# ishine/TargetDiarization

Measured on AMD Instinct MI355X. Metric: real-time factor (audio-sec/wall-sec) full infer() pipe, 16kHz mono, 1/2/4/8 GPU, higher is better.
Workload: dtype f32 (split-f16 x3: fp32-accurate products from three f16 MFMA passes, fp32 accumulate); 1 GPU; BASELINE configs[3]: 1800 s synthetic conversation (two alternating speakers, 20 % overlap) = 180 x 10 s windows: MossFormer2 (90 windows per launch) -> loudness swap -> ERes2NetV2 on every 10 s window of both streams + cosine vs a target embedding -> Paraformer (SANM encoder, CIF predictor, NAR decoder, argmax tokens + timestamps) on 30 s segments of both streams -> CT-Transformer punctuation of ; windows_per_launch=90

## Files before the change

### targetdiarization_amd/csrc/gemm_h3.hpp

```cpp
#pragma once
#include <cstdio>
#include <cstdlib>
#include <typeinfo>
#include <vector>
#include <hip/hip_runtime.h>
#include <stdint.h>

#include "devutil.hpp"
#include "gemm.hpp"

namespace tdx {

typedef _Float16 f16x8 __attribute__((ext_vector_type(8)));

constexpr int H3_BM = 256, H3_BN = 256, H3_BK = 16, H3_THREADS = 512;
constexpr int H3_ROWB = 64;
constexpr int H3_OPER = 256 * H3_ROWB;
constexpr int H3_STAGE = 2 * H3_OPER;
constexpr int H3_NBUF = 4;
constexpr int H3_AUX_AHEAD = 3;
constexpr int H3_LDS = H3_NBUF * H3_STAGE;
constexpr int H3_LDS_EXTRA = 12288;

struct H3Seg {
    const unsigned char* A;
    const unsigned char* B;
    const float* sa;
    const float* sb;
    long lda, ldb;
    long strideA, strideB, strideA2, strideB2;
    long strideSA, strideSB, strideSA2, strideSB2;
    int sa_mul, sb_mul;
    int K;
    int zdiv;
    int kchunk, ktotal;
    int segk;
    long strideSeg;
    int a_shift, a_period;
    const unsigned char* a_zero;
};

struct H3Args {
    H3Seg seg[2];
    int nseg;
    int M, N;
    int tiles_m, tiles_n;
    int map_mode, mp, gw, batches;
    int mc;
    int pair_off;
    int cv_Hin, cv_Win, cv_Hout, cv_Wout, cv_stride, cv_ntaps, cv_cin;
    int cv_taps_total;
    const unsigned char* zero_row;
    int dbg;
    unsigned long long* stamps;
};

#ifdef TDX_H3_STAMPS
#define H3_STAMP(i) do { if (g.stamps && threadIdx.x == 0) g.stamps[(long)blockIdx.x * 8 + (i)] = wall_clock64(); } while (0)
#define H3_STAMP_HW() do { if (g.stamps && threadIdx.x == 0) g.stamps[(long)blockIdx.x * 8 + 7] = \
    (unsigned long long)__builtin_amdgcn_s_getreg((31 << 11) | 4) | ((unsigned long long)__builtin_amdgcn_s_getreg((31 << 11) | 20) << 32); } while (0)
#else
#define H3_STAMP(i) do {} while (0)
#define H3_STAMP_HW() do {} while (0)
#endif

inline H3Seg h3_seg(const void* A, const float* sa, long lda, const void* B, const float* sb, long ldb, int K) {
    H3Seg s{};
    s.A = (const unsigned char*)A; s.B = (const unsigned char*)B; s.sa = sa; s.sb = sb; s.lda = lda; s.ldb = ldb; s.K = K; s.zdiv = 1;
    s.sa_mul = 1; s.sb_mul = 1;
    return s;
}

__device__ __forceinline__ void h3_glds16(const unsigned char* g, unsigned char* l) {
    __builtin_amdgcn_global_load_lds((const __attribute__((address_space(1))) void*)g, (__attribute__((address_space(3))) void*)l, 16, 0, 0);
}

typedef __fp16 h3_fp16x4 __attribute__((__vector_size__(4 * sizeof(__fp16))));
typedef _Float16 f16x4 __attribute__((ext_vector_type(4)));

template <bool TR>
__device__ __forceinline__ f16x8 h3_frag(const unsigned char* p) {
    if constexpr (!TR) {
        return *reinterpret_cast<const f16x8*>(p);
    } else {
        const h3_fp16x4 lo = __builtin_amdgcn_ds_read_tr16_b64_v4f16((__attribute__((address_space(3))) h3_fp16x4*)p);
        const h3_fp16x4 hi = __builtin_amdgcn_ds_read_tr16_b64_v4f16((__attribute__((address_space(3))) h3_fp16x4*)(p + 4096));
        f16x8 r;
#pragma unroll
        for (int i = 0; i < 4; ++i) { r[i] = (_Float16)lo[i]; r[4 + i] = (_Float16)hi[i]; }
        return r;
    }
}

struct H3TrRaw { uint2 lo, hi; };
__device__ __forceinline__ unsigned h3_lds_addr(const unsigned char* p) {
    return (unsigned)(size_t)(__attribute__((address_space(3))) const unsigned char*)p;
}
template <int OFF>
__device__ __forceinline__ void h3_tr_read(H3TrRaw& r, unsigned a) {
    asm volatile("ds_read_b64_tr_b16 %0, %1 offset:%2" : "=v"(r.lo) : "v"(a), "n"(OFF) : "memory");
    asm volatile("ds_read_b64_tr_b16 %0, %1 offset:%2" : "=v"(r.hi) : "v"(a), "n"(OFF + 4096) : "memory");
}
__device__ __forceinline__ f16x8 h3_tr_value(const H3TrRaw& r) {
    typedef unsigned u4 __attribute__((ext_vector_type(4)));
    return __builtin_bit_cast(f16x8, u4{r.lo.x, r.lo.y, r.hi.x, r.hi.y});
}
template <int N>
__device__ __forceinline__ void h3_tr_fence(H3TrRaw (&r)[N]) {
    static_assert(N == 2 || N == 4 || N == 8, "fence over 2, 4 or 8 raw fragments");
    if constexpr (N == 8)
        asm volatile("s_waitcnt lgkmcnt(0)" : "+v"(r[0].lo), "+v"(r[0].hi), "+v"(r[1].lo), "+v"(r[1].hi), "+v"(r[2].lo), "+v"(r[2].hi), "+v"(r[3].lo), "+v"(r[3].hi),
                     "+v"(r[4].lo), "+v"(r[4].hi), "+v"(r[5].lo), "+v"(r[5].hi), "+v"(r[6].lo), "+v"(r[6].hi), "+v"(r[7].lo), "+v"(r[7].hi) :: "memory");
    else if constexpr (N == 4)
        asm volatile("s_waitcnt lgkmcnt(0)" : "+v"(r[0].lo), "+v"(r[0].hi), "+v"(r[1].lo), "+v"(r[1].hi), "+v"(r[2].lo), "+v"(r[2].hi), "+v"(r[3].lo), "+v"(r[3].hi) :: "memory");
    else
        asm volatile("s_waitcnt lgkmcnt(0)" : "+v"(r[0].lo), "+v"(r[0].hi), "+v"(r[1].lo), "+v"(r[1].hi) :: "memory");
}
// ... 116 lines not shown
        const _Float16 a = (_Float16)xs;
        hi[i] = a;
        lo[i] = (_Float16)(xs - (float)a);
    }
    *reinterpret_cast<f16x8*>(dst) = hi;
    *reinterpret_cast<f16x8*>(dst + 16) = lo;
}

struct H3Pair { uint2 hi, lo; };
__device__ __forceinline__ H3Pair h3_split4(float4 v, float s) {
    typedef _Float16 h4 __attribute__((ext_vector_type(4)));
    const float xs[4] = {v.x * s, v.y * s, v.z * s, v.w * s};
    h4 a, b;
#pragma unroll
    for (int j = 0; j < 4; ++j) { const _Float16 t = (_Float16)xs[j]; a[j] = t; b[j] = (_Float16)(xs[j] - (float)t); }
    H3Pair r;
    r.hi = __builtin_bit_cast(uint2, a); r.lo = __builtin_bit_cast(uint2, b);
    return r;
}
__device__ __forceinline__ uint4 h3_pair16(int q, float4 v, float s) {
    const H3Pair o = h3_split4(v, s);
    const bool odd = q & 1;
    const uint2 send = odd ? o.hi : o.lo;
    uint2 recv;
    recv.x = (unsigned)__builtin_amdgcn_mov_dpp((int)send.x, 0xB1, 0xF, 0xF, true);
    recv.y = (unsigned)__builtin_amdgcn_mov_dpp((int)send.y, 0xB1, 0xF, 0xF, true);
    return odd ? make_uint4(recv.x, recv.y, o.lo.x, o.lo.y) : make_uint4(o.hi.x, o.hi.y, recv.x, recv.y);
}
__device__ __forceinline__ void h3_emit4(unsigned char* prow, int q, float4 v, float s) {
    *reinterpret_cast<uint4*>(prow + (q >> 1) * 32 + ((q & 1) ? 16 : 0)) = h3_pair16(q, v, s);
}
__device__ __forceinline__ void h3_emit4_pred(unsigned char* prow, int q, float4 v, float s, bool ok) {
    const uint4 w = h3_pair16(q, v, s);
    if (ok) *reinterpret_cast<uint4*>(prow + (q >> 1) * 32 + ((q & 1) ? 16 : 0)) = w;
}
__device__ __forceinline__ float h3_absmax4(float4 v) { return fmaxf(fmaxf(fabsf(v.x), fabsf(v.y)), fmaxf(fabsf(v.z), fabsf(v.w))); }


struct H3PlOut { unsigned char* planes; long pitch; float* scale; float* ss; long seg_stride; };
template <class E, class = void> struct epi_has_plout { static constexpr bool value = false; };
template <class E> struct epi_has_plout<E, decltype((void)&E::plout, void())> { static constexpr bool value = true; };
template <class E, class = void> struct epi_has_rowout { static constexpr bool value = false; };
template <class E> struct epi_has_rowout<E, decltype((void)&E::rowout, void())> { static constexpr bool value = true; };
struct H3Conv {
    const float* w; int wld;
    int ncols;
    unsigned char* planes; long pitch;
    float sv;
    float* u32; int u0; long ld32;
    int S, Sp;
};
template <class E, class = void> struct epi_has_conv { static constexpr bool value = false; };
template <class E> struct epi_has_conv<E, decltype((void)&E::conv, void())> { static constexpr bool value = true; };
constexpr int H3_CONV_STEP = 240, H3_CONV_HALO = 8;
template <class T> __device__ __forceinline__ void h3_assume_row(const T&) {}
__device__ __forceinline__ void h3_assume_row(long rw) { __builtin_assume(rw >= 0); }

template <bool A_TR, bool B_TR, bool PAIRED, bool TWOSEG, class Epi, int VARIANT = 0, bool A_CONV = false>
__global__ __launch_bounds__(H3_THREADS, 2) void gemm_h3_kernel(H3Args g, Epi epi) {
    static_assert(!A_CONV || (!A_TR && !TWOSEG), "A_CONV: row-major A planes, one weight segment");
    constexpr bool PINGPONG = VARIANT == 5;
    extern __shared__ __attribute__((aligned(1024))) unsigned char lds[];
    const int tid = threadIdx.x;
    const int lane = tid & 63, wave = tid >> 6;
    const int l31 = lane & 31, h = lane >> 5;
    const int wm = wave >> 2, wn = wave & 3;

    int z, bm, bn;
    {
        const int x = blockIdx.x & 7, i = blockIdx.x >> 3;
        if (g.map_mode == 0) {
            z = blockIdx.y;
            int i2 = i, mbase = 0, mcur = g.mp;
            if (g.mc > 0) { const int tpc = g.mc * g.tiles_n, c = i / tpc; i2 = i - c * tpc; mbase = c * g.mc; mcur = min(g.mc, g.mp - mbase); }
            const int per = mcur * g.gw, ngf = g.tiles_n / g.gw;
            const int p = i2 / per;
            int lm, n;
            if (p < ngf) { const int j = i2 - p * per; lm = j / g.gw; n = p * g.gw + (j - lm * g.gw); }
            else { const int rem = g.tiles_n - ngf * g.gw; const int j = i2 - ngf * per; lm = j / rem; n = ngf * g.gw + (j - lm * rem); }
            bm = x * g.mp + mbase + lm; bn = n;
            if (bm >= g.tiles_m) return;
        } else {
            const int tpb = g.tiles_m * g.tiles_n;
            const int zb = i / tpb, tt = i - zb * tpb;
            z = zb * 8 + x;
            if (z >= g.batches) return;
            bm = tt / g.tiles_n; bn = tt - bm * g.tiles_n;
        }
    }
    constexpr bool CONV = epi_has_conv<Epi>::value;
    static_assert(!CONV || (!PAIRED && !A_TR && !B_TR && !A_CONV && epi_has_ptr<Epi>::value && epi_has_rowmul<Epi>::value), "CONV: row-major Linear with a put_scaled() functor");
    const int m0 = CONV ? bm * H3_CONV_STEP - H3_CONV_HALO : bm * H3_BM;
    const int n0 = PAIRED ? bn * (H3_BN / 2) : bn * H3_BN;
    H3_STAMP(0); H3_STAMP_HW();

    f32x16 acc[4][2];
#pragma unroll
    for (int i = 0; i < 4; ++i)
#pragma unroll
        for (int j = 0; j < 2; ++j)
#pragma unroll
            for (int r = 0; r < 16; ++r) acc[i][j][r] = 0.f;

    const bool stB = wave >= 4;
    const int sdst = (stB ? H3_OPER : 0) + (wave & 3) * 4096;
    H3Frag f;
    {
        const int fl = (l31 >> 2) & 3;
        const int q = (lane >> 2) & 3, p4 = lane & 3, nb = (lane >> 4) & 1;
        f.a0 = (wm * 128 + l31) * H3_ROWB;
        f.apl[0] = ((2 * h) ^ fl) << 4; f.apl[1] = ((2 * h + 1) ^ fl) << 4;
#pragma unroll
        for (int tm = 0; tm < 4; ++tm) f.at[tm] = (8 * h + q) * 1024 + wm * 512 + (((tm ^ q) << 6) + nb * 32 + p4 * 8);
        if constexpr (B_TR) f.b0 = H3_OPER + (8 * h + q) * 1024 + (((wn ^ q) << 6) + nb * 32 + p4 * 8);
        else f.b0 = H3_OPER + (wn * 32 + l31) * H3_ROWB;
        f.bpl[0] = f.apl[0]; f.bpl[1] = f.apl[1];
    }
    const bool full_n = PAIRED || (n0 + 128 < g.N);
    const bool wave_on = m0 + wm * 128 < g.M;

    auto setup = [&](const H3Seg& sg, const unsigned char* (&gp)[4], long& gstep) {
        const int z1 = z / sg.zdiv, z2 = z - z1 * sg.zdiv;
        if (!stB) {
            const unsigned char* Ag = sg.A + (long)z1 * sg.strideA + (long)z2 * sg.strideA2;
            if constexpr (!A_TR) {
                gstep = H3_ROWB;
#pragma unroll
                for (int j = 0; j < 4; ++j) {
                    const int r = (wave & 3) * 64 + (lane >> 2) + 16 * j;
                    const int mr = min(max(m0 + r, 0), g.M - 1);
                    const unsigned char* rowp = Ag + (long)(mr + sg.a_shift) * sg.lda;
                    if (sg.a_period && (mr % sg.a_period) == 0) rowp = sg.a_zero;
                    gp[j] = rowp + (((lane & 3) ^ ((r >> 2) & 3)) << 4);
                }
            } else {
                gstep = 16 * sg.lda;
                const int blk = min(m0 / 128 + (lane >> 5), (g.M - 1) / 128);
#pragma unroll
                for (int j = 0; j < 4; ++j)
                    {
                    const int ch = (lane & 15) ^ (j << 2);
                    gp[j] = Ag + (long)((wave & 3) * 4 + j) * sg.lda + blk * 512 + (ch >> 2) * 128 + ((lane >> 4) & 1) * 64 + (ch & 3) * 16;
                }
            }
        } else {
            const unsigned char* Bg = sg.B + (long)z1 * sg.strideB + (long)z2 * sg.strideB2;
            if constexpr (!B_TR) {
// ... 43 lines not shown
    RowT* rwl = reinterpret_cast<RowT*>(lds + H3_LDS + 2048);
    float sa_own = 0.f;
    RowT rw_own{};
    if (tid < 256) {
        sa_own = (sl.sa + (long)zl1 * sl.strideSA + (long)zl2 * sl.strideSA2 + (sl.segk ? (long)(sl.K / sl.segk - 1) * sl.strideSeg : 0L))[(long)min(max(m0 + tid, 0), g.M - 1) * sl.sa_mul];
        if constexpr (HAS_ROW) rw_own = epi.row(z, min(max(m0 + tid, 0), g.M - 1));
        if constexpr (epi_has_rowmul<Epi>::value) sa_own *= epi.rowmul(rw_own);
    }

    const H3Seg& sg0 = g.seg[0];
    const int zz2 = z % sg0.zdiv;
    const int nkt0 = (sg0.kchunk ? max(0, min(sg0.K, sg0.ktotal - zz2 * sg0.kchunk)) : sg0.K) / H3_BK;
    const int nkt = TWOSEG ? nkt0 + g.seg[1].K / H3_BK : nkt0;
    if (nkt > 0) {
        const unsigned char* gp[4];
        long gstep;
        setup(sg0, gp, gstep);
        if constexpr (A_CONV) { if (!stB) setup_conv(0, gp); }
        if constexpr (TWOSEG) {
            const H3Seg& s1 = g.seg[1];
            const float* sa0 = sg0.sa + (long)(z / sg0.zdiv) * sg0.strideSA + (long)zz2 * sg0.strideSA2;
            const float* sa1 = s1.sa + (long)(z / s1.zdiv) * s1.strideSA + (long)(z % s1.zdiv) * s1.strideSA2;
            if (tid < 256) {
                const int m = min(max(m0 + tid, 0), g.M - 1);
                const bool zr = sg0.a_period && (m % sg0.a_period) == 0;
                const float f0 = zr ? 1.0f : sa0[(long)(m + sg0.a_shift) * sg0.sa_mul];
                reinterpret_cast<float*>(lds + H3_LDS)[tid] = f0 / sa1[(long)m * s1.sa_mul];
            }
        }

        if constexpr (!TWOSEG && !A_TR) {
            if (sg0.segk && tid < 256) {
                const float* sab = sg0.sa + (long)(z / sg0.zdiv) * sg0.strideSA + (long)zz2 * sg0.strideSA2 + (long)min(m0 + tid, g.M - 1) * sg0.sa_mul;
                float* rft = reinterpret_cast<float*>(lds + H3_LDS + 4096);
                const int nb = sg0.K / sg0.segk - 1;
                float sc[8];
#pragma unroll
                for (int j = 0; j < 8; ++j) sc[j] = sab[(long)min(j, nb) * sg0.strideSeg];
#pragma unroll
                for (int j = 0; j < 7; ++j)
                    if (j < nb) rft[j * 256 + tid] = sc[j] / sc[j + 1];
            }
        }

#pragma unroll
        for (int p = 0; p < 4; ++p)
            if (p < nkt0) {
#pragma unroll
                for (int j = 0; j < 4; ++j) h3_glds16(gp[j] + p * gstep, lds + p * H3_STAGE + sdst + j * 1024);
            }
        if (tid < 256) { sal[tid] = sa_own; if constexpr (HAS_ROW) rwl[tid] = rw_own; }
        if (nkt0 >= 4) H3_WAIT_VM(12); else if (nkt0 == 3) H3_WAIT_VM(8); else if (nkt0 == 2) H3_WAIT_VM(4); else H3_WAIT_VM(0);
        H3_BARRIER();
        H3_STAMP(1);
        f16x8 ah[4], al[4], bh[2], bl[2];
#pragma unroll
        for (int tn = 0; tn < 2; ++tn) {
            bh[tn] = h3_frag<B_TR>(h3_addr_b<B_TR>(lds, f, tn, 0));
            bl[tn] = h3_frag<B_TR>(h3_addr_b<B_TR>(lds, f, tn, 1));
        }
#pragma unroll
        for (int tm = 0; tm < 4; ++tm) {
            ah[tm] = h3_frag<A_TR>(h3_addr_a<A_TR>(lds, f, tm, 0));
            al[tm] = h3_frag<A_TR>(h3_addr_a<A_TR>(lds, f, tm, 1));
        }

#define H3_STEADY(FULLN, PH, LIMIT, TILE0)                                                                             \
            for (; t + 4 < (LIMIT); ++t) {                                                                             \
                if constexpr (!TWOSEG && !A_TR && !A_CONV) {                                                           \
                    if (t == seg_bnd) {     \
                        const float* rfl = reinterpret_cast<const float*>(lds + H3_LDS + 4096) + seg_j * 256;          \
                        _Pragma("unroll") for (int tm = 0; tm < 4; ++tm)                                               \
                            _Pragma("unroll") for (int j = 0; j < 4; ++j) {                                            \
                                const f32x4 rf = *reinterpret_cast<const f32x4*>(rfl + wm * 128 + tm * 32 + 8 * j + 4 * h); \
                                _Pragma("unroll") for (int i = 0; i < 4; ++i) {                                        \
                                    acc[tm][0][4 * j + i] *= rf[i];                                                    \
                                    acc[tm][1][4 * j + i] *= rf[i];                                                    \
                                }                                                                                      \
                            }                                                                                          \
                        ++seg_j; seg_bnd += seg_stp;                                                                   \
                    }                                                                                                  \
                }                                                                                                      \
                if (VARIANT != 9) H3_WAIT_VM(8);                                                                       \
                if (VARIANT != 4) H3_BARRIER();                                                                        \
                if (wave_on)                                                                                           \
                    h3_stage<A_TR, B_TR, FULLN, VARIANT != 2 && VARIANT != 3, VARIANT != 1 && VARIANT != 3, PH, VARIANT == 6>( \
                        acc, ah, al, bh, bl, lds + ((t + 1) & 3) * H3_STAGE, f, gp, (long)(t + 4 - (TILE0)) * gstep,   \
                        lds + ((t + 4) & 3) * H3_STAGE + sdst);                                                        \
                else                                                                                                   \
                    h3_stage_dma_only<VARIANT != 1 && VARIANT != 3>(gp, (long)(t + 4 - (TILE0)) * gstep,               \
                                                                    lds + ((t + 4) & 3) * H3_STAGE + sdst);            \
            }
#define H3_RUN(FULLN, PH)                                                                                              \
        {                                                                                                              \
            int t = 0;                                                                                                 \
             \
            const int seg_stp = sg0.segk ? sg0.segk / H3_BK : 0;                                                       \
            int seg_bnd = sg0.segk ? seg_stp : 0x7fffffff, seg_j = 0;                                                  \
            (void)seg_stp; (void)seg_bnd; (void)seg_j;                                                                 \
            if constexpr (TWOSEG) {                                                                                    \
                H3_STEADY(FULLN, PH, nkt0, 0)                                                                          \
                setup(g.seg[1], gp, gstep);                                                                            \
                H3_STEADY(FULLN, PH, nkt0 + 4, nkt0)                                                                   \
                {                                                                                                      \
                    const H3Seg& s1 = g.seg[1];                                                                        \
                    const float* sb0 = sg0.sb + (long)(z / sg0.zdiv) * sg0.strideSB + (long)zz2 * sg0.strideSB2;       \
                    const float* sb1 = s1.sb + (long)(z / s1.zdiv) * s1.strideSB + (long)(z % s1.zdiv) * s1.strideSB2; \
// ... 51 lines not shown
                    }
            };
            auto frags = [&](const unsigned char* st, auto fulln) {
                constexpr bool FN = decltype(fulln)::value;
#pragma unroll
                for (int tn = 0; tn < (FN ? 2 : 1); ++tn) {
                    bh[tn] = h3_frag<B_TR>(h3_addr_b<B_TR>(st, f, tn, 0));
                    bl[tn] = h3_frag<B_TR>(h3_addr_b<B_TR>(st, f, tn, 1));
                }
#pragma unroll
                for (int tm = 0; tm < 4; ++tm) {
                    ah[tm] = h3_frag<A_TR>(h3_addr_a<A_TR>(st, f, tm, 0));
                    al[tm] = h3_frag<A_TR>(h3_addr_a<A_TR>(st, f, tm, 1));
                }
            };
            auto dma = [&](int ti) {
#pragma unroll
                for (int j = 0; j < 4; ++j) h3_glds16(gp[j] + (long)ti * gstep, lds + (ti & 3) * H3_STAGE + sdst + j * 1024);
            };
            auto run = [&](auto fulln) {
                for (int t = 0; t < nkt; ++t) {
                    if (!stB) {
                        const int last = min(t + 3, nkt - 1);
                        wait_keep(last - t);
                        H3_BARRIER();
                        if (wave_on) mma(fulln);
                        wait_keep(last - (t + 1));
                        H3_BARRIER();
                        if (t + 1 < nkt && wave_on) frags(lds + ((t + 1) & 3) * H3_STAGE, fulln);
                        if (t + 4 < nkt) dma(t + 4);
                    } else {
                        wait_keep(min(max(t + 2, 3), nkt - 1) - t);
                        H3_BARRIER();
                        if (t > 0 && wave_on) frags(lds + (t & 3) * H3_STAGE, fulln);
                        if (t >= 1 && t + 3 < nkt) dma(t + 3);
                        wait_keep(min(max(t + 3, 3), nkt - 1) - (t + 1));
                        H3_BARRIER();
                        if (wave_on) mma(fulln);
                    }
                }
            };
            if (full_n) run(std::true_type{}); else run(std::false_type{});
        } else {
        if (full_n) { if (stB) H3_RUN(true, 1) else H3_RUN(true, 0) }
        else { if (stB) H3_RUN(false, 1) else H3_RUN(false, 0) }
        }
#undef H3_RUN
#undef H3_STEADY
    } else {
        if (tid < 256) { sal[tid] = sa_own; if constexpr (HAS_ROW) rwl[tid] = rw_own; }
        __syncthreads();
    }

    H3_STAMP(2);
    if (g.dbg & 1) {
        float x = 0.f;
#pragma unroll
        for (int r = 0; r < 16; ++r) x += acc[0][0][r] + acc[1][1][r] + acc[2][0][r] + acc[3][1][r];
        if (x != 123.456f) return;
    }
    const float* sb = sl.sb + (long)zl1 * sl.strideSB + (long)zl2 * sl.strideSB2;
    const int sbm = sl.sb_mul;
    const int lrow0 = wm * 128 + 4 * h, lcol0 = wn * 32 + l31;
    auto row_of = [&](int lr) -> RowT { if constexpr (HAS_ROW) return rwl[lr]; else return RowT{}; };
    auto epilogue = [&](auto tag) {
        if constexpr (!epi_has_plout<Epi>::value) {
        constexpr bool CHECK = decltype(tag)::value;
        int lrow = lrow0, lcol = lcol0;
        asm volatile("" : "+v"(lrow), "+v"(lcol));
        auto rowm = [&](int lr) { return CHECK ? min(m0 + lr, g.M - 1) : m0 + lr; };
        if constexpr (PAIRED) {
            const int c = n0 + lcol;
            auto cc = epi.col(z, c);
            float sc0 = sb[(long)c * sbm], sc1 = sb[(long)(g.pair_off + c) * sbm];
            touch(cc); touch(sc0); touch(sc1);
            if constexpr (epi_has_pairmul<Epi>::value) { const float2 pm = epi.pairmul(cc); sc0 *= pm.x; sc1 *= pm.y; }
            if constexpr (epi_has_aux<Epi>::value) {
                constexpr int AH = H3_AUX_AHEAD;
                decltype(epi.aux(0, 0, 0, RowT{})) ax[AH + 1][8];
                auto fetch = [&](int hb) {
                    int lb = lrow + (hb >> 1) * 32;
                    asm volatile("" : "+v"(lb));
#pragma unroll
                    for (int r8 = 0; r8 < 8; ++r8) {
                        const int r = (hb & 1) * 8 + r8;
                        const int lr = lb + (r & 3) + 8 * (r >> 2);
                        ax[hb % (AH + 1)][r8] = epi.aux(z, rowm(lr), c, row_of(lr));
                    }
                };
#pragma unroll
                for (int hb = 0; hb < AH; ++hb) fetch(hb);
#pragma unroll
                for (int hb = 0; hb < 8; ++hb) {
                    __builtin_amdgcn_sched_barrier(0);
                    if (hb + AH < 8) fetch(hb + AH);
                    RowT rw[8];
                    float sr[8];
                    int lb = lrow + (hb >> 1) * 32;
                    asm volatile("" : "+v"(lb));
#pragma unroll
                    for (int r8 = 0; r8 < 8; ++r8) {
                        const int r = (hb & 1) * 8 + r8;
                        const int lr = lb + (r & 3) + 8 * (r >> 2);
                        rw[r8] = row_of(lr);
                        sr[r8] = sal[lr];
                    }
#pragma unroll
// ... 129 lines not shown
        asm volatile("" : "+v"(lrow), "+v"(lcol));
        float* const T = reinterpret_cast<float*>(lds);
        const H3PlOut po = epi.plout(z);
        auto rowm = [&](int lr) { return CHECK ? min(m0 + lr, g.M - 1) : m0 + lr; };
        __syncthreads();
        if constexpr (PAIRED) {
            static_assert(epi_has_aux<Epi>::value && epi_has_pairmul<Epi>::value, "PLOUT PAIRED: gate-style functor");
            const int c = n0 + lcol;
            auto cc = epi.col(z, c);
            float sc0 = sb[(long)c * sbm], sc1 = sb[(long)(g.pair_off + c) * sbm];
            touch(cc); touch(sc0); touch(sc1);
            { const float2 pm = epi.pairmul(cc); sc0 *= pm.x; sc1 *= pm.y; }
            constexpr int AH = H3_AUX_AHEAD;
            decltype(epi.aux(0, 0, 0, RowT{})) ax[AH + 1][8];
            auto fetch = [&](int hb) {
                int lb = lrow + (hb >> 1) * 32;
                asm volatile("" : "+v"(lb));
#pragma unroll
                for (int r8 = 0; r8 < 8; ++r8) {
                    const int r = (hb & 1) * 8 + r8;
                    const int lr = lb + (r & 3) + 8 * (r >> 2);
                    ax[hb % (AH + 1)][r8] = epi.aux(z, rowm(lr), c, row_of(lr));
                }
            };
#pragma unroll
            for (int hb = 0; hb < AH; ++hb) fetch(hb);
#pragma unroll
            for (int hb = 0; hb < 8; ++hb) {
                __builtin_amdgcn_sched_barrier(0);
                if (hb + AH < 8) fetch(hb + AH);
                RowT rw[8];
                float sr[8];
                int lb = lrow + (hb >> 1) * 32;
                asm volatile("" : "+v"(lb));
#pragma unroll
                for (int r8 = 0; r8 < 8; ++r8) {
                    const int r = (hb & 1) * 8 + r8;
                    const int lr = lb + (r & 3) + 8 * (r >> 2);
                    rw[r8] = row_of(lr);
                    sr[r8] = sal[lr];
                }
#pragma unroll
                for (int r8 = 0; r8 < 8; ++r8) touch(ax[hb % (AH + 1)][r8]);
#pragma unroll
                for (int r8 = 0; r8 < 8; ++r8) {
                    const int tm = hb >> 1, r = (hb & 1) * 8 + r8;
                    const int lr = lb + (r & 3) + 8 * (r >> 2);
                    float v = epi.val2_scaled(z, m0 + lr, c, acc[tm][0][r] * (sr[r8] * sc0), acc[tm][1][r] * (sr[r8] * sc1), rw[r8], cc, ax[hb % (AH + 1)][r8]);
                    if (CHECK && m0 + lr >= g.M) v = 0.f;
                    T[lr * 128 + (lcol ^ (((lr >> 2) & 1) << 5))] = v;
                }
            }
            __syncthreads();
            H3_STAMP(3);
            const int hw = lane >> 5, l32 = lane & 31;
            unsigned char* const pbase = po.planes + (long)n0 * 4;
#pragma unroll 4
            for (int it = 0; it < 16; ++it) {
                const int rl = wave * 32 + it * 2 + hw;
                const int m = m0 + rl;
                const long pr = (!CHECK || m < g.M) ? epi.prow(z, min(m, g.M - 1)) : -1L;
                const f32x4 v4 = *reinterpret_cast<const f32x4*>(T + rl * 128 + ((4 * l32) ^ (((rl >> 2) & 1) << 5)));
                const float4 v = make_float4(v4[0], v4[1], v4[2], v4[3]);
                const float mu = h3_half_max(h3_absmax4(v));
                const float q2 = h3_half_sum((v.x * v.x + v.y * v.y) + (v.z * v.z + v.w * v.w));
                float inv;
                const float sc = h3_row_scale(mu, inv);
                h3_emit4_pred(pbase + (pr < 0 ? 0 : pr) * po.pitch, l32, v, sc, pr >= 0);
                if (l32 == 0 && pr >= 0) {
                    po.scale[(long)bn * po.seg_stride + pr] = inv;
                    if (po.ss) po.ss[(long)bn * po.seg_stride + pr] = q2;
                }
            }
        } else {
            int nn[2];
            decltype(epi.col(0, 0)) cc[2];
            float sc[2];
#pragma unroll
            for (int tn = 0; tn < 2; ++tn) {
                nn[tn] = n0 + tn * 128 + lcol;
                cc[tn] = epi.col(z, nn[tn]);
                sc[tn] = sb[(long)nn[tn] * sbm];
            }
            touch(cc[0]); touch(cc[1]); touch(sc[0]); touch(sc[1]);
            unsigned char* const pbase = po.planes + (long)n0 * 4;
            auto phase2 = [&](int hf) {
                __syncthreads();
#pragma unroll 4
                for (int it = 0; it < 16; ++it) {
                    const int rl = wave * 16 + it;
                    const int lr = (rl >> 6) * 128 + (2 * hf + ((rl >> 5) & 1)) * 32 + (rl & 31);
                    const int m = m0 + lr;
                    const long pr = (!CHECK || m < g.M) ? epi.prow(z, min(m, g.M - 1)) : -1L;
                    const f32x4 v4 = *reinterpret_cast<const f32x4*>(T + rl * 256 + ((4 * lane) ^ (((rl >> 2) & 1) << 5)));
                    const float4 v = make_float4(v4[0], v4[1], v4[2], v4[3]);
                    const float mu = wave_max(h3_absmax4(v));
                    float q2 = (v.x * v.x + v.y * v.y) + (v.z * v.z + v.w * v.w);
                    if (po.ss) q2 = h3_wave_sum(q2);
                    float inv;
                    const float s_ = h3_row_scale(mu, inv);
                    if (pr >= 0) {
                        h3_emit4(pbase + pr * po.pitch, lane, v, s_);
                        if constexpr (epi_has_rowout<Epi>::value) *reinterpret_cast<f32x4*>(epi.rowout(z, pr, n0) + 4 * lane) = v4;
                        if (lane == 0) {
                            po.scale[(long)bn * po.seg_stride + pr] = inv;
                            if (po.ss) po.ss[(long)bn * po.seg_stride + pr] = q2;
                        }
// ... 28 lines not shown
                    asm volatile("" : "+v"(lb));
#pragma unroll
                    for (int r8 = 0; r8 < 8; ++r8) {
                        const int r = half * 8 + r8;
                        const int lr = lb + (r & 3) + 8 * (r >> 2);
                        rw[r8] = row_of(lr);
                        sr[r8] = sal[lr];
                    }
#pragma unroll
                    for (int r8 = 0; r8 < 8; ++r8) touch(ax[i % (AH + 1)][r8]);
#pragma unroll
                    for (int r8 = 0; r8 < 8; ++r8) {
                        const int r = half * 8 + r8;
                        const int lr = lb + (r & 3) + 8 * (r >> 2);
                        float v = 0.f;
                        if (!CHECK || m0 + lr < g.M) v = epi.val(z, m0 + lr, nn[tn], acc[tm][tn][r] * (sr[r8] * sc[tn]), rw[r8], cc[tn], ax[i % (AH + 1)][r8]);
                        const int rl = lr - wm * 64 - (tm - tmh) * 32;
                        T[rl * 256 + ((tn * 128 + lcol) ^ (((rl >> 2) & 1) << 5))] = v;
                    }
                    if (i == 7 || i == 15) phase2(i >> 3);
                }
            } else {
#pragma unroll
                for (int hf = 0; hf < 2; ++hf) {
                    if (hf) __syncthreads();
#pragma unroll
                    for (int tn = 0; tn < 2; ++tn) {
#pragma unroll
                        for (int tmh = 0; tmh < 2; ++tmh) {
                            const int tm = 2 * hf + tmh;
#pragma unroll
                            for (int r = 0; r < 16; ++r) {
                                const int lr = lrow + tm * 32 + (r & 3) + 8 * (r >> 2);
                                const RowT rw = row_of(lr);
                                const float sr = sal[lr];
                                float v = 0.f;
                                if (!CHECK || m0 + lr < g.M) v = epi.val(z, m0 + lr, nn[tn], acc[tm][tn][r] * (sr * sc[tn]), rw, cc[tn]);
                                const int rl = lr - wm * 64 - hf * 64 + 0 * tmh;
                                T[rl * 256 + ((tn * 128 + lcol) ^ (((rl >> 2) & 1) << 5))] = v;
                            }
                        }
                    }
                    phase2(hf);
                }
            }
        }
        }
    };

    auto epilogue_conv = [&]() {
        if constexpr (CONV) {
        int lrow = lrow0, lcol = lcol0;
        asm volatile("" : "+v"(lrow), "+v"(lcol));
        const H3Conv cv = epi.conv();
        int nn[2];
        decltype(epi.col(0, 0)) cc[2];
        float sc[2];
#pragma unroll
        for (int tn = 0; tn < 2; ++tn) {
            nn[tn] = n0 + tn * 128 + lcol;
            const int nc = min(nn[tn], g.N - 1);
            cc[tn] = epi.col(z, nc);
            sc[tn] = sb[(long)nc * sbm] * epi.colmul(cc[tn]);
        }
        touch(cc[0]); touch(cc[1]); touch(sc[0]); touch(sc[1]);
        if (n0 >= cv.ncols) {
#pragma unroll
            for (int tn = 0; tn < 2; ++tn) {
                if (nn[tn] >= g.N) continue;
                float* const p0 = epi.ptr(z, m0 + lrow, nn[tn]);
                const long ldm = epi.ldm();
#pragma unroll
                for (int tm = 0; tm < 4; ++tm) {
#pragma unroll
                    for (int r = 0; r < 16; ++r) {
                        const int k = tm * 32 + (r & 3) + 8 * (r >> 2);
                        const int lr = lrow + k;
                        const RowT rw = row_of(lr);
                        const float sr = sal[lr];
                        if (lr >= H3_CONV_HALO && lr < H3_CONV_HALO + H3_CONV_STEP && m0 + lr < g.M)
                            epi.put_scaled(p0 + k * ldm, acc[tm][tn][r] * (sr * sc[tn]), rw, cc[tn]);
                    }
                }
            }
            return;
        }
        float* const T = reinterpret_cast<float*>(lds);
        int* const sid = reinterpret_cast<int*>(lds + H3_LDS + 4096);
        const bool fast = m0 >= 0 && m0 + 255 < g.M && (m0 / cv.S) == ((m0 + 255) / cv.S);
        if (!fast && tid < 256) { const int m = m0 + tid; sid[tid] = (m >= 0 && m < g.M) ? m / cv.S : -1; }
        typedef float v2f __attribute__((ext_vector_type(2)));
        constexpr int KT = 17, HALF = 8, RW = 30;
        const int r_first = H3_CONV_HALO + RW * wave;
        __syncthreads();
        auto half = [&](auto tnc) {
            constexpr int tn = decltype(tnc)::value;
#pragma unroll
            for (int tm = 0; tm < 4; ++tm) {
#pragma unroll
                for (int j = 0; j < 4; ++j) {
                    const int lr = lrow + tm * 32 + 8 * j;
                    const f32x4 sr4 = *reinterpret_cast<const f32x4*>(sal + lr);
#pragma unroll
                    for (int i = 0; i < 4; ++i) T[(lr + i) * 128 + lcol] = (g.dbg & 16) ? acc[tm][tn][4 * j + i] : epi.act(acc[tm][tn][4 * j + i] * (sr4[i] * sc[tn]), cc[tn]);
                }
            }
            const int colp = n0 + tn * 128 + 2 * lane;
            v2f w[KT];
#pragma unroll
            for (int t = 0; t < KT; ++t) w[t] = *reinterpret_cast<const v2f*>(cv.w + (long)t * cv.wld + colp);
            __syncthreads();
            H3_STAMP(tn == 0 ? 3 : 6);
            const float* const Tc = T + 2 * lane;
            const unsigned poff = (unsigned)((colp >> 5) * 128 + (colp & 31) * 2);
            const bool has32 = cv.u32 && colp >= cv.u0;
            const unsigned uoff = (unsigned)(colp - cv.u0) * 4u;
            auto emit = [&](v2f o, long prow, long m) {
                typedef _Float16 h2 __attribute__((ext_vector_type(2)));
                const v2f xs = o * v2f{cv.sv, cv.sv};
                const h2 hi = h2{(_Float16)xs[0], (_Float16)xs[1]};
                const h2 lo = h2{(_Float16)(xs[0] - (float)hi[0]), (_Float16)(xs[1] - (float)hi[1])};
                unsigned char* const rowp = cv.planes + prow * cv.pitch;
                if (g.dbg & 4) { if (xs[0] == 123.456f) *reinterpret_cast<h2*>(rowp + poff) = lo; return; }
                *reinterpret_cast<h2*>(rowp + poff) = hi;
                *reinterpret_cast<h2*>(rowp + 64 + poff) = lo;
                if (has32) *reinterpret_cast<v2f*>(reinterpret_cast<unsigned char*>(cv.u32 + m * cv.ld32) + uoff) = o;
            };
            if (fast) {
                const int b0 = m0 / cv.S;
                const long prow0 = (long)b0 * cv.Sp + (m0 - b0 * cv.S);
                constexpr int RUN = 10;
#pragma unroll 1
                for (int r0 = r_first; r0 < r_first + RW; r0 += RUN) {
                    v2f win[RUN + KT - 1];
#pragma unroll
                    for (int i = 0; i < RUN + KT - 1; ++i) win[i] = *reinterpret_cast<const v2f*>(Tc + (r0 - HALF + i) * 128);
#pragma unroll
                    for (int i = 0; i < RUN; ++i) {
                        v2f o = win[HALF + i];
                        if (!(g.dbg & 8)) {
#pragma unroll
                            for (int t = 0; t < KT; ++t) o = __builtin_elementwise_fma(w[t], win[i + t], o);
                        }
                        emit(o, prow0 + r0 + i, (long)m0 + r0 + i);
                    }
                }
            } else {
#pragma unroll 1
                for (int lr = r_first; lr < r_first + RW; ++lr) {
                    const int so = sid[lr];
                    if (so < 0) continue;
                    v2f o = *reinterpret_cast<const v2f*>(Tc + lr * 128);
#pragma unroll
                    for (int t = 0; t < KT; ++t) {
                        const int rt = lr + t - HALF;
                        if (sid[rt] == so) o = __builtin_elementwise_fma(w[t], *reinterpret_cast<const v2f*>(Tc + rt * 128), o);
                    }
                    const long m = (long)m0 + lr;
                    emit(o, (long)so * cv.Sp + (m - (long)so * cv.S), m);
                }
            }
        };
        if (g.dbg & 32) return;
        half(std::integral_constant<int, 0>{});
        H3_STAMP(5);
        __syncthreads();
        half(std::integral_constant<int, 1>{});
        }
    };
    if constexpr (CONV) { epilogue_conv(); H3_STAMP(4); return; }
    bool whole = m0 + 256 <= g.M;
    if constexpr (epi_has_full<Epi>::value) whole = whole && epi.full(z, m0);
    if constexpr (epi_has_plout<Epi>::value) { if (whole) epilogue_pl(std::false_type{}); else epilogue_pl(std::true_type{}); }
    else { if (whole) epilogue(std::false_type{}); else epilogue(std::true_type{}); }
    H3_STAMP(4);
}

template <bool A_TR, bool B_TR, bool PAIRED, bool TWOSEG, class Epi, int VARIANT = 0, bool A_CONV = false>
inline hipError_t launch_gemm_h3x(H3Args g, int batches, Epi epi, hipStream_t st) {
    static const hipError_t attr_rc = hipFuncSetAttribute(reinterpret_cast<const void*>(&gemm_h3_kernel<A_TR, B_TR, PAIRED, TWOSEG, Epi, VARIANT, A_CONV>), hipFuncAttributeMaxDynamicSharedMemorySize,
                            H3_LDS + H3_LDS_EXTRA);
    (void)attr_rc;
    g.tiles_m = (g.M + H3_BM - 1) / H3_BM;
    if constexpr (epi_has_conv<Epi>::value) {
        g.tiles_m = (g.M + H3_CONV_STEP - 1) / H3_CONV_STEP;
        if (batches != 1 || g.seg[0].segk || g.seg[0].kchunk) return hipErrorInvalidValue;
    }
    g.tiles_n = PAIRED ? g.N / (H3_BN / 2) : (g.N + H3_BN - 1) / H3_BN;
    g.batches = batches;
    dim3 grid;
    if (g.tiles_m >= 16 && batches <= 4) {
        g.map_mode = 0;
        g.mp = (g.tiles_m + 7) / 8;
        long ktot = 0;
        for (int i = 0; i < g.nseg; ++i) ktot += g.seg[i].K;
        static const long gw_kb = [] { const char* e = getenv("TDX_H3_GW_KB"); return e ? atol(e) : 1536L; }();
        long gw = (gw_kb * 1024) / (256L * ktot * 4);
        if (gw < 1) gw = 1;
        if (gw > g.tiles_n) gw = g.tiles_n;
        g.gw = (int)gw;
        static const int mc_env = [] { const char* e = getenv("TDX_H3_MC"); return e ? atoi(e) : -1; }();
        g.mc = 0;
        if (g.gw < g.tiles_n) {
            long mc = mc_env >= 0 ? mc_env : (6L * 1024 * 1024) / (256L * ktot * 4);
            if (mc > 0 && mc < g.mp) g.mc = (int)mc;
        }
        grid = dim3(8 * g.mp * g.tiles_n, batches, 1);
    } else {
        g.map_mode = 1;
        g.mp = 0; g.gw = 1;
        grid = dim3(8 * ((batches + 7) / 8) * g.tiles_m * g.tiles_n, 1, 1);
    }
    if (TWOSEG && (g.seg[0].K < 64 || g.seg[1].K < 64 || g.seg[0].kchunk || g.seg[1].kchunk)) return hipErrorInvalidValue;
    for (int i = 0; i < g.nseg; ++i) {
        const H3Seg& sg = g.seg[i];
        if (sg.segk && (TWOSEG || A_TR || A_CONV || sg.segk % 64 || sg.K % sg.segk || sg.K / sg.segk > 8 || sg.kchunk)) return hipErrorInvalidValue;
        if ((sg.a_shift || sg.a_period) && (A_TR || A_CONV || (sg.a_period && !sg.a_zero))) return hipErrorInvalidValue;
    }
    if (epi_has_plout<Epi>::value && !PAIRED && g.N % 256) return hipErrorInvalidValue;
    if (A_CONV && (g.cv_cin < 64 || g.cv_cin % 16 || g.seg[0].K != g.cv_ntaps * g.cv_cin || !g.zero_row ||
                   batches != (g.cv_taps_total ? g.cv_taps_total / g.cv_ntaps : 1) || (g.cv_taps_total && g.cv_taps_total % g.cv_ntaps))) return hipErrorInvalidValue;
    static const int dbg = [] { const char* e = getenv("TDX_H3_DEBUG"); return e ? atoi(e) : 0; }();
    g.dbg = dbg;
#ifdef TDX_H3_STAMPS
    static int stamp_calls = 0;
    const long nblk = (long)grid.x * grid.y;
    if (!g.stamps && getenv("TDX_H3_STAMPS_DIR") && nblk >= 512 && ++stamp_calls == 4) {
        unsigned long long* buf = nullptr;
        hipMalloc((void**)&buf, nblk * 64);
        hipMemsetAsync(buf, 0, nblk * 64, st);
        g.stamps = buf;
        g.tiles_n = g.tiles_n;
        hipLaunchKernelGGL((gemm_h3_kernel<A_TR, B_TR, PAIRED, TWOSEG, Epi, VARIANT, A_CONV>), grid, dim3(H3_THREADS), H3_LDS + H3_LDS_EXTRA, st, g, epi);
        hipStreamSynchronize(st);
        std::vector<unsigned long long> hbuf(nblk * 8);
        hipMemcpy(hbuf.data(), buf, nblk * 64, hipMemcpyDeviceToHost);
        long ktot = 0;
        for (int i = 0; i < g.nseg; ++i) ktot += g.seg[i].K;
        char fn[512];
        snprintf(fn, sizeof fn, "%s/h3_%s_M%d_N%d_K%ld_z%d.bin", getenv("TDX_H3_STAMPS_DIR"), typeid(Epi).name(), g.M, g.N, ktot, batches);
        if (FILE* f = fopen(fn, "wb")) { fwrite(hbuf.data(), 8, hbuf.size(), f); fclose(f); }
        hipFree(buf);
        return hipGetLastError();
    }
#endif
    hipLaunchKernelGGL((gemm_h3_kernel<A_TR, B_TR, PAIRED, TWOSEG, Epi, VARIANT, A_CONV>), grid, dim3(H3_THREADS), H3_LDS + H3_LDS_EXTRA, st, g, epi);
    return hipGetLastError();
}

template <bool PAIRED, class Epi, int VARIANT = 0>
inline hipError_t launch_gemm_h3(H3Args g, int batches, Epi epi, hipStream_t st) {
    return launch_gemm_h3x<false, false, PAIRED, false, Epi, VARIANT>(g, batches, epi, st);
}


template <int UNUSED = 0>
__global__ __launch_bounds__(256) void h3_split_rows_kernel(const float* __restrict__ x, long ld, unsigned char* __restrict__ planes,
                                                           float* __restrict__ scale, long R, int K, int Kp) {
    const int lane = threadIdx.x & 63;
    const long row = (long)blockIdx.x * 4 + (threadIdx.x >> 6);
    if (row >= R) return;
    const float* xr = x + row * ld;
    float v[4][8];
    float mu = 0.f;
    const int nch = Kp / 8;
#pragma unroll
    for (int c = 0; c < 4; ++c) {
        const int ch = lane + 64 * c;
#pragma unroll
        for (int i = 0; i < 8; ++i) v[c][i] = 0.f;
        if (ch * 8 < K) {
            const f32x4 a = ldg4(xr + ch * 8), b = ldg4(xr + ch * 8 + 4);
#pragma unroll
            for (int i = 0; i < 4; ++i) { v[c][i] = a[i]; v[c][4 + i] = b[i]; }
        }
#pragma unroll
        for (int i = 0; i < 8; ++i) mu = fmaxf(mu, fabsf(v[c][i]));
    }
#pragma unroll
    for (int o = 32; o >= 1; o >>= 1) mu = fmaxf(mu, __shfl_xor(mu, o, 64));
    float inv;
    const float s = h3_row_scale(mu, inv);
    unsigned char* pr = planes + row * (long)Kp * 4;
#pragma unroll
    for (int c = 0; c < 4; ++c) {
        const int ch = lane + 64 * c;
        if (ch < nch) h3_store_chunk(pr + ch * 32, v[c], s);
    }
    if (lane == 0) scale[row] = inv;
}

template <int UNUSED = 0>
__global__ __launch_bounds__(256) void h3_split_rows_static_kernel(const float* __restrict__ x, long ld, unsigned char* __restrict__ planes,
                                                                  long R, int K, int Kp, float s) {
    const long i = (long)blockIdx.x * 256 + threadIdx.x;
    const int per = Kp / 8;
    if (i >= R * per) return;
    const long row = i / per;
    const int ch = (int)(i - row * per);
// ... 91 lines not shown
```

Baseline: 504.4 audio-s/s.

## Process conv-fused GEMM as multi-tile strips carrying halo rows in LDS

The conv-fused GEMM epilogue used to give each block one 256-row tile that advanced by 240 rows, recomputing a 16-row halo per tile. Each block now walks a strip of up to R consecutive 256-row tiles (default 4). It carries the last 16 tile rows into an extra LDS buffer so the next tile's depthwise conv can read its left context without recomputation. This removes the halo GEMM work and cuts the number of blocks. In exchange it adds LDS footprint and serial tiles per block, which reduces parallelism for small M, and it also changes the M-grouping heuristic.

```diff
diff --git a/targetdiarization_amd/csrc/gemm_h3.hpp b/targetdiarization_amd/csrc/gemm_h3.hpp
--- a/targetdiarization_amd/csrc/gemm_h3.hpp
+++ b/targetdiarization_amd/csrc/gemm_h3.hpp
@@ -52,17 +52,22 @@
     int cv_taps_total;
     const unsigned char* zero_row;
     int dbg;
+    int conv_strip;
     unsigned long long* stamps;
 };
 
 #ifdef TDX_H3_STAMPS
-#define H3_STAMP(i) do { if (g.stamps && threadIdx.x == 0) g.stamps[(long)blockIdx.x * 8 + (i)] = wall_clock64(); } while (0)
-#define H3_STAMP_HW() do { if (g.stamps && threadIdx.x == 0) g.stamps[(long)blockIdx.x * 8 + 7] = \
+#define H3_STAMP_AT(rec, i) do { if (g.stamps && threadIdx.x == 0) g.stamps[(long)(rec) * 8 + (i)] = wall_clock64(); } while (0)
+#define H3_STAMP_HW_AT(rec) do { if (g.stamps && threadIdx.x == 0) g.stamps[(long)(rec) * 8 + 7] = \
     (unsigned long long)__builtin_amdgcn_s_getreg((31 << 11) | 4) | ((unsigned long long)__builtin_amdgcn_s_getreg((31 << 11) | 20) << 32); } while (0)
 #else
-#define H3_STAMP(i) do {} while (0)
-#define H3_STAMP_HW() do {} while (0)
+#define H3_STAMP_AT(rec, i) do {} while (0)
+#define H3_STAMP_HW_AT(rec) do {} while (0)
 #endif
+#define H3_STAMP(i) H3_STAMP_AT(blockIdx.x, i)
+#define H3_STAMP_HW() H3_STAMP_HW_AT(blockIdx.x)
+#define H3_STAMPT(i) H3_STAMP_AT(stamp_rec, i)
+#define H3_STAMPT_HW() H3_STAMP_HW_AT(stamp_rec)
 
 inline H3Seg h3_seg(const void* A, const float* sa, long lda, const void* B, const float* sb, long ldb, int K) {
     H3Seg s{};
@@ -285,7 +290,17 @@
 };
 template <class E, class = void> struct epi_has_conv { static constexpr bool value = false; };
 template <class E> struct epi_has_conv<E, decltype((void)&E::conv, void())> { static constexpr bool value = true; };
-constexpr int H3_CONV_STEP = 240, H3_CONV_HALO = 8;
+constexpr int H3_CONV_HALO = 8;
+constexpr int H3_CONV_CARRY_ROWS = 2 * H3_CONV_HALO;
+constexpr int H3_CONV_CARRY = 2 * H3_CONV_CARRY_ROWS * 128 * 4;
+constexpr int H3_CONV_STRIP_MAX = 64;
+static_assert(H3_LDS + H3_LDS_EXTRA + H3_CONV_CARRY <= 160 * 1024, "ring + extras + carry must fit the 160 KiB of a CU");
+__host__ __device__ constexpr int h3_conv_strip_rows(int R) { return H3_BM * R - 2 * H3_CONV_HALO; }
+__host__ __device__ constexpr int h3_conv_strips(int M, int R) { return (M + h3_conv_strip_rows(R) - 1) / h3_conv_strip_rows(R); }
+__host__ __device__ constexpr int h3_conv_strip_tiles(int M, int R, int s) {
+    const int n = (M - s * h3_conv_strip_rows(R) + 2 * H3_CONV_HALO + H3_BM - 1) / H3_BM;
+    return n < R ? n : R;
+}
 template <class T> __device__ __forceinline__ void h3_assume_row(const T&) {}
 __device__ __forceinline__ void h3_assume_row(long rw) { __builtin_assume(rw >= 0); }
 
@@ -294,16 +309,16 @@
     static_assert(!A_CONV || (!A_TR && !TWOSEG), "A_CONV: row-major A planes, one weight segment");
     constexpr bool PINGPONG = VARIANT == 5;
     extern __shared__ __attribute__((aligned(1024))) unsigned char lds[];
-    const int tid = threadIdx.x;
-    const int lane = tid & 63, wave = tid >> 6;
-    const int l31 = lane & 31, h = lane >> 5;
-    const int wm = wave >> 2, wn = wave & 3;
-
-    int z, bm, bn;
+    const int tid_ = threadIdx.x;
+    const int lane_ = tid_ & 63, wave_ = tid_ >> 6;
+    const int l31_ = lane_ & 31, h_ = lane_ >> 5;
+    const int wm_ = wave_ >> 2, wn_ = wave_ & 3;
+
+    int z_, bm, bn;
     {
         const int x = blockIdx.x & 7, i = blockIdx.x >> 3;
         if (g.map_mode == 0) {
-            z = blockIdx.y;
+            z_ = blockIdx.y;
             int i2 = i, mbase = 0, mcur = g.mp;
             if (g.mc > 0) { const int tpc = g.mc * g.tiles_n, c = i / tpc; i2 = i - c * tpc; mbase = c * g.mc; mcur = min(g.mc, g.mp - mbase); }
             const int per = mcur * g.gw, ngf = g.tiles_n / g.gw;
@@ -316,16 +331,27 @@
         } else {
             const int tpb = g.tiles_m * g.tiles_n;
             const int zb = i / tpb, tt = i - zb * tpb;
-            z = zb * 8 + x;
-            if (z >= g.batches) return;
+            z_ = zb * 8 + x;
+            if (z_ >= g.batches) return;
             bm = tt / g.tiles_n; bn = tt - bm * g.tiles_n;
         }
     }
     constexpr bool CONV = epi_has_conv<Epi>::value;
     static_assert(!CONV || (!PAIRED && !A_TR && !B_TR && !A_CONV && epi_has_ptr<Epi>::value && epi_has_rowmul<Epi>::value), "CONV: row-major Linear with a put_scaled() functor");
-    const int m0 = CONV ? bm * H3_CONV_STEP - H3_CONV_HALO : bm * H3_BM;
-    const int n0 = PAIRED ? bn * (H3_BN / 2) : bn * H3_BN;
-    H3_STAMP(0); H3_STAMP_HW();
+    const int strip_m0 = CONV ? bm * h3_conv_strip_rows(g.conv_strip) - H3_CONV_HALO : bm * H3_BM;
+    const int n0_ = PAIRED ? bn * (H3_BN / 2) : bn * H3_BN;
+    const int ntile = CONV ? h3_conv_strip_tiles(g.M, g.conv_strip, bm) : 1;
+    int tj = 0;
+    do {
+    int tid = tid_, z = z_, n0 = n0_;
+    if constexpr (CONV) asm volatile("" : "+v"(tid), "+s"(z), "+s"(n0));
+    const int lane = CONV ? tid & 63 : lane_, wave = CONV ? tid >> 6 : wave_;
+    const int l31 = CONV ? lane & 31 : l31_, h = CONV ? lane >> 5 : h_;
+    const int wm = CONV ? wave >> 2 : wm_, wn = CONV ? wave & 3 : wn_;
+    const int m0 = CONV ? strip_m0 + tj * H3_BM : strip_m0;
+    const long stamp_rec = CONV ? (long)blockIdx.x * g.conv_strip + tj : (long)blockIdx.x;
+    (void)stamp_rec;
+    H3_STAMPT(0); H3_STAMPT_HW();
 
     f32x16 acc[4][2];
 #pragma unroll
@@ -475,7 +501,7 @@
         if (tid < 256) { sal[tid] = sa_own; if constexpr (HAS_ROW) rwl[tid] = rw_own; }
         if (nkt0 >= 4) H3_WAIT_VM(12); else if (nkt0 == 3) H3_WAIT_VM(8); else if (nkt0 == 2) H3_WAIT_VM(4); else H3_WAIT_VM(0);
         H3_BARRIER();
-        H3_STAMP(1);
+        H3_STAMPT(1);
         f16x8 ah[4], al[4], bh[2], bl[2];
 #pragma unroll
         for (int tn = 0; tn < 2; ++tn) {
@@ -633,7 +659,7 @@
         __syncthreads();
     }
 
-    H3_STAMP(2);
+    H3_STAMPT(2);
     if (g.dbg & 1) {
         float x = 0.f;
 #pragma unroll
@@ -869,7 +895,7 @@
                 }
             }
             __syncthreads();
-            H3_STAMP(3);
+            H3_STAMPT(3);
             const int hw = lane >> 5, l32 = lane & 31;
             unsigned char* const pbase = po.planes + (long)n0 * 4;
 #pragma unroll 4
@@ -1004,7 +1030,8 @@
         if constexpr (CONV) {
         int lrow = lrow0, lcol = lcol0;
         asm volatile("" : "+v"(lrow), "+v"(lcol));
-        const H3Conv cv = epi.conv();
+        H3Conv cv = epi.conv();
+        asm volatile("" : "+s"(cv.wld));
         int nn[2];
         decltype(epi.col(0, 0)) cc[2];
         float sc[2];
@@ -1016,12 +1043,15 @@
             sc[tn] = sb[(long)nc * sbm] * epi.colmul(cc[tn]);
         }
         touch(cc[0]); touch(cc[1]); touch(sc[0]); touch(sc[1]);
+        const bool first = tj == 0, last = tj + 1 == ntile;
         if (n0 >= cv.ncols) {
+            const int own_lo = first ? H3_CONV_HALO : 0, own_hi = last ? H3_BM - H3_CONV_HALO : H3_BM;
 #pragma unroll
             for (int tn = 0; tn < 2; ++tn) {
                 if (nn[tn] >= g.N) continue;
                 float* const p0 = epi.ptr(z, m0 + lrow, nn[tn]);
-                const long ldm = epi.ldm();
+                long ldm = epi.ldm();
+                asm volatile("" : "+s"(ldm));
 #pragma unroll
                 for (int tm = 0; tm < 4; ++tm) {
 #pragma unroll
@@ -1030,20 +1060,24 @@
                         const int lr = lrow + k;
                         const RowT rw = row_of(lr);
                         const float sr = sal[lr];
-                        if (lr >= H3_CONV_HALO && lr < H3_CONV_HALO + H3_CONV_STEP && m0 + lr < g.M)
+                        if (lr >= own_lo && lr < own_hi && m0 + lr < g.M)
                             epi.put_scaled(p0 + k * ldm, acc[tm][tn][r] * (sr * sc[tn]), rw, cc[tn]);
                     }
                 }
             }
             return;
         }
+        constexpr int CR = H3_CONV_CARRY_ROWS;
         float* const T = reinterpret_cast<float*>(lds);
-        int* const sid = reinterpret_cast<int*>(lds + H3_LDS + 4096);
-        const bool fast = m0 >= 0 && m0 + 255 < g.M && (m0 / cv.S) == ((m0 + 255) / cv.S);
-        if (!fast && tid < 256) { const int m = m0 + tid; sid[tid] = (m >= 0 && m < g.M) ? m / cv.S : -1; }
+        float* const carry = reinterpret_cast<float*>(lds + H3_LDS + H3_LDS_EXTRA);
+        int* const sid = reinterpret_cast<int*>(lds + H3_LDS + 4096) + CR;
+        const int mlo = first ? m0 : m0 - CR;
+        const bool fast = mlo >= 0 && m0 + 255 < g.M && (mlo / cv.S) == ((m0 + 255) / cv.S);
+        if (!fast && tid < 256 + CR) { const int m = m0 - CR + tid; sid[tid - CR] = (m >= 0 && m < g.M) ? m / cv.S : -1; }
         typedef float v2f __attribute__((ext_vector_type(2)));
-        constexpr int KT = 17, HALF = 8, RW = 30;
-        const int r_first = H3_CONV_HALO + RW * wave;
+        constexpr int KT = 17, HALF = 8;
+        const int r_first = first ? H3_CONV_HALO + 30 * wave : -H3_CONV_HALO + 32 * wave;
+        const int r_count = first ? 30 : 32;
         __syncthreads();
         auto half = [&](auto tnc) {
             constexpr int tn = decltype(tnc)::value;
@@ -1062,8 +1096,9 @@
 #pragma unroll
             for (int t = 0; t < KT; ++t) w[t] = *reinterpret_cast<const v2f*>(cv.w + (long)t * cv.wld + colp);
             __syncthreads();
-            H3_STAMP(tn == 0 ? 3 : 6);
+            H3_STAMPT(tn == 0 ? 3 : 6);
             const float* const Tc = T + 2 * lane;
+            float* const Cc = carry + tn * (CR * 128) + 2 * lane;
             const unsigned poff = (unsigned)((colp >> 5) * 128 + (colp & 31) * 2);
             const bool has32 = cv.u32 && colp >= cv.u0;
             const unsigned uoff = (unsigned)(colp - cv.u0) * 4u;
@@ -1079,63 +1114,101 @@
                 if (has32) *reinterpret_cast<v2f*>(reinterpret_cast<unsigned char*>(cv.u32 + m * cv.ld32) + uoff) = o;
             };
             if (fast) {
-                const int b0 = m0 / cv.S;
+                const int b0 = mlo / cv.S;
                 const long prow0 = (long)b0 * cv.Sp + (m0 - b0 * cv.S);
-                constexpr int RUN = 10;
+                auto runs = [&](auto runc, auto carc) {
+                    constexpr int RUN = decltype(runc)::value;
+                    constexpr bool CARRIED = decltype(carc)::value;
 #pragma unroll 1
-                for (int r0 = r_first; r0 < r_first + RW; r0 += RUN) {
-                    v2f win[RUN + KT - 1];
-#pragma unroll
-                    for (int i = 0; i < RUN + KT - 1; ++i) win[i] = *reinterpret_cast<const v2f*>(Tc + (r0 - HALF + i) * 128);
-#pragma unroll
-                    for (int i = 0; i < RUN; ++i) {
-                        v2f o = win[HALF + i];
-                        if (!(g.dbg & 8)) {
-#pragma unroll
-                            for (int t = 0; t < KT; ++t) o = __builtin_elementwise_fma(w[t], win[i + t], o);
+                    for (int r0 = r_first; r0 < r_first + r_count; r0 += RUN) {
+                        v2f win[RUN + KT - 1];
+                        if (CARRIED && r0 < 0) {
+                            static_assert(!CARRIED || RUN == HALF, "wave 0's first two runs start at tile rows -8 and 0");
+#pragma unroll
+                            for (int i = 0; i < RUN + KT - 1; ++i)
+                                win[i] = *reinterpret_cast<const v2f*>(i < CR ? Cc + i * 128 : Tc + (i - CR) * 128);
+                        } else if (CARRIED && r0 < HALF) {
+#pragma unroll
+                            for (int i = 0; i < RUN + KT - 1; ++i)
+                                win[i] = *reinterpret_cast<const v2f*>(i < HALF ? Cc + (HALF + i) * 128 : Tc + (i - HALF) * 128);
+                        } else {
+#pragma unroll
+                            for (int i = 0; i < RUN + KT - 1; ++i) win[i] = *reinterpret_cast<const v2f*>(Tc + (r0 - HALF + i) * 128);
                         }
-                        emit(o, prow0 + r0 + i, (long)m0 + r0 + i);
-                    }
-                }
+#pragma unroll
+                        for (int i = 0; i < RUN; ++i) {
+                            v2f o = win[HALF + i];
+                            if (!(g.dbg & 8)) {
+#pragma unroll
+                                for (int t = 0; t < KT; ++t) o = __builtin_elementwise_fma(w[t], win[i + t], o);
+                            }
+                            emit(o, prow0 + r0 + i, (long)m0 + r0 + i);
+                        }
+                    }
+                };
+                if (first) runs(std::integral_constant<int, 10>{}, std::false_type{});
+                else runs(std::integral_constant<int, 8>{}, std::true_type{});
             } else {
+                auto trow = [&](int r) -> const float* { return r < 0 ? Cc + (r + CR) * 128 : Tc + r * 128; };
 #pragma unroll 1
-                for (int lr = r_first; lr < r_first + RW; ++lr) {
+                for (int lr = r_first; lr < r_first + r_count; ++lr) {
                     const int so = sid[lr];
                     if (so < 0) continue;
-                    v2f o = *reinterpret_cast<const v2f*>(Tc + lr * 128);
+                    v2f o = *reinterpret_cast<const v2f*>(trow(lr));
 #pragma unroll
                     for (int t = 0; t < KT; ++t) {
                         const int rt = lr + t - HALF;
-                        if (sid[rt] == so) o = __builtin_elementwise_fma(w[t], *reinterpret_cast<const v2f*>(Tc + rt * 128), o);
+                        if (sid[rt] == so) o = __builtin_elementwise_fma(w[t], *reinterpret_cast<const v2f*>(trow(rt)), o);
                     }
                     const long m = (long)m0 + lr;
                     emit(o, (long)so * cv.Sp + (m - (long)so * cv.S), m);
                 }
+            }
+            if (!last && wave == 0) {
+                v2f cr[CR];
+#pragma unroll
+                for (int i = 0; i < CR; ++i) cr[i] = *reinterpret_cast<const v2f*>(Tc + (H3_BM - CR + i) * 128);
+#pragma unroll
+                for (int i = 0; i < CR; ++i) *reinterpret_cast<v2f*>(Cc + i * 128) = cr[i];
             }
         };
         if (g.dbg & 32) return;
         half(std::integral_constant<int, 0>{});
-        H3_STAMP(5);
+        H3_STAMPT(5);
         __syncthreads();
         half(std::integral_constant<int, 1>{});
         }
     };
-    if constexpr (CONV) { epilogue_conv(); H3_STAMP(4); return; }
+    if constexpr (CONV) {
+        epilogue_conv();
+        H3_STAMPT(4);
+        if (++tj >= ntile) return;
+        __syncthreads();
+        continue;
+    } else {
     bool whole = m0 + 256 <= g.M;
     if constexpr (epi_has_full<Epi>::value) whole = whole && epi.full(z, m0);
     if constexpr (epi_has_plout<Epi>::value) { if (whole) epilogue_pl(std::false_type{}); else epilogue_pl(std::true_type{}); }
     else { if (whole) epilogue(std::false_type{}); else epilogue(std::true_type{}); }
-    H3_STAMP(4);
+    H3_STAMPT(4);
+    return;
+    }
+    } while (true);
 }
 
 template <bool A_TR, bool B_TR, bool PAIRED, bool TWOSEG, class Epi, int VARIANT = 0, bool A_CONV = false>
 inline hipError_t launch_gemm_h3x(H3Args g, int batches, Epi epi, hipStream_t st) {
+    constexpr int lds_bytes = H3_LDS + H3_LDS_EXTRA + (epi_has_conv<Epi>::value ? H3_CONV_CARRY : 0);
     static const hipError_t attr_rc = hipFuncSetAttribute(reinterpret_cast<const void*>(&gemm_h3_kernel<A_TR, B_TR, PAIRED, TWOSEG, Epi, VARIANT, A_CONV>), hipFuncAttributeMaxDynamicSharedMemorySize,
-                            H3_LDS + H3_LDS_EXTRA);
+                            lds_bytes);
     (void)attr_rc;
     g.tiles_m = (g.M + H3_BM - 1) / H3_BM;
+    int strip = 1;
     if constexpr (epi_has_conv<Epi>::value) {
-        g.tiles_m = (g.M + H3_CONV_STEP - 1) / H3_CONV_STEP;
+        static const int strip_env = [] { const char* e = getenv("TDX_H3_CONV_STRIP"); return e ? atoi(e) : 4; }();
+        strip = strip_env < 1 ? 1 : strip_env > H3_CONV_STRIP_MAX ? H3_CONV_STRIP_MAX : strip_env;
+        g.tiles_m = h3_conv_strips(g.M, 1);
+        g.conv_strip = strip;
         if (batches != 1 || g.seg[0].segk || g.seg[0].kchunk) return hipErrorInvalidValue;
     }
     g.tiles_n = PAIRED ? g.N / (H3_BN / 2) : (g.N + H3_BN - 1) / H3_BN;
@@ -1143,6 +1216,7 @@
     dim3 grid;
     if (g.tiles_m >= 16 && batches <= 4) {
         g.map_mode = 0;
+        if constexpr (epi_has_conv<Epi>::value) g.tiles_m = h3_conv_strips(g.M, strip);
         g.mp = (g.tiles_m + 7) / 8;
         long ktot = 0;
         for (int i = 0; i < g.nseg; ++i) ktot += g.seg[i].K;
@@ -1155,11 +1229,13 @@
         g.mc = 0;
         if (g.gw < g.tiles_n) {
             long mc = mc_env >= 0 ? mc_env : (6L * 1024 * 1024) / (256L * ktot * 4);
+            if (mc_env < 0 && strip > 1) mc = mc / strip > 0 ? mc / strip : 1;
             if (mc > 0 && mc < g.mp) g.mc = (int)mc;
         }
         grid = dim3(8 * g.mp * g.tiles_n, batches, 1);
     } else {
         g.map_mode = 1;
+        if constexpr (epi_has_conv<Epi>::value) g.tiles_m = h3_conv_strips(g.M, strip);
         g.mp = 0; g.gw = 1;
         grid = dim3(8 * ((batches + 7) / 8) * g.tiles_m * g.tiles_n, 1, 1);
     }
@@ -1176,27 +1252,27 @@
     g.dbg = dbg;
 #ifdef TDX_H3_STAMPS
     static int stamp_calls = 0;
-    const long nblk = (long)grid.x * grid.y;
+    const long nblk = (long)grid.x * grid.y * strip;
     if (!g.stamps && getenv("TDX_H3_STAMPS_DIR") && nblk >= 512 && ++stamp_calls == 4) {
         unsigned long long* buf = nullptr;
         hipMalloc((void**)&buf, nblk * 64);
         hipMemsetAsync(buf, 0, nblk * 64, st);
         g.stamps = buf;
         g.tiles_n = g.tiles_n;
-        hipLaunchKernelGGL((gemm_h3_kernel<A_TR, B_TR, PAIRED, TWOSEG, Epi, VARIANT, A_CONV>), grid, dim3(H3_THREADS), H3_LDS + H3_LDS_EXTRA, st, g, epi);
+        hipLaunchKernelGGL((gemm_h3_kernel<A_TR, B_TR, PAIRED, TWOSEG, Epi, VARIANT, A_CONV>), grid, dim3(H3_THREADS), lds_bytes, st, g, epi);
         hipStreamSynchronize(st);
         std::vector<unsigned long long> hbuf(nblk * 8);
         hipMemcpy(hbuf.data(), buf, nblk * 64, hipMemcpyDeviceToHost);
         long ktot = 0;
         for (int i = 0; i < g.nseg; ++i) ktot += g.seg[i].K;
         char fn[512];
-        snprintf(fn, sizeof fn, "%s/h3_%s_M%d_N%d_K%ld_z%d.bin", getenv("TDX_H3_STAMPS_DIR"), typeid(Epi).name(), g.M, g.N, ktot, batches);
+        snprintf(fn, sizeof fn, "%s/h3_%s_M%d_N%d_K%ld_z%d_R%d.bin", getenv("TDX_H3_STAMPS_DIR"), typeid(Epi).name(), g.M, g.N, ktot, batches, strip);
         if (FILE* f = fopen(fn, "wb")) { fwrite(hbuf.data(), 8, hbuf.size(), f); fclose(f); }
         hipFree(buf);
         return hipGetLastError();
     }
 #endif
-    hipLaunchKernelGGL((gemm_h3_kernel<A_TR, B_TR, PAIRED, TWOSEG, Epi, VARIANT, A_CONV>), grid, dim3(H3_THREADS), H3_LDS + H3_LDS_EXTRA, st, g, epi);
+    hipLaunchKernelGGL((gemm_h3_kernel<A_TR, B_TR, PAIRED, TWOSEG, Epi, VARIANT, A_CONV>), grid, dim3(H3_THREADS), lds_bytes, st, g, epi);
     return hipGetLastError();
 }
 
```

After: 502.2 audio-s/s. About the same (-0.4%).
